# keep-starknet-strange/frieda

Measured on AMD Instinct MI355X. Metric: M31 field-elems/s committed (NTT+FRI+Merkle), higher is better.
Workload: dtype u32

## Files before the change

frieda_amd/csrc/clock_stamps.h:

```cpp
#pragma once

#ifdef FRIEDA_CLOCK_STAMPS
#define FR_CLOCK_SLOTS 16384
#define FR_CLOCK_DECL(name) __device__ unsigned long long name[4 * FR_CLOCK_SLOTS];
#define FR_CLOCK_BEGIN(tie)                                                                                                        \
    unsigned long long cs_c0_, cs_r0_;                                                                                             \
    asm volatile("s_memtime %0\n\ts_memrealtime %1\n\ts_waitcnt lgkmcnt(0)" : "=s"(cs_c0_), "=s"(cs_r0_)::"memory"); \
    asm volatile("" : "+v"(tie) : "s"(cs_c0_));
#define FR_CLOCK_END(buf, tie)                                                                                                     \
    {                                                                                                                              \
        asm volatile("" ::"v"(tie));                                                                                               \
        unsigned long long cs_c1_, cs_r1_;                                                                                         \
        asm volatile("s_memtime %0\n\ts_memrealtime %1\n\ts_waitcnt lgkmcnt(0)" : "=s"(cs_c1_), "=s"(cs_r1_)::"memory"); \
        if (threadIdx.x == 0 && blockIdx.y == 0 && blockIdx.z == 0 && blockIdx.x < FR_CLOCK_SLOTS) {                              \
            buf[4 * blockIdx.x + 0] = cs_c0_;                                                                                      \
            buf[4 * blockIdx.x + 1] = cs_r0_;                                                                                      \
            buf[4 * blockIdx.x + 2] = cs_c1_;                                                                                      \
            buf[4 * blockIdx.x + 3] = cs_r1_;                                                                                      \
        }                                                                                                                          \
    }
#define FR_CLOCK_READER(fn, buf)                                                                                                   \
    extern "C" int fn(unsigned long long* out, unsigned long n_words) {                                                            \
        const size_t bytes = sizeof(unsigned long long) * (n_words < 4 * FR_CLOCK_SLOTS ? n_words : 4 * FR_CLOCK_SLOTS);          \
        return hipMemcpyFromSymbol(out, HIP_SYMBOL(buf), bytes, 0, hipMemcpyDeviceToHost) == hipSuccess ? 0 : 1;                   \
    }
#else
#define FR_CLOCK_DECL(name)
#define FR_CLOCK_BEGIN(tie)
#define FR_CLOCK_END(buf, tie)
#define FR_CLOCK_READER(fn, buf)
#endif
```

frieda_amd/csrc/context.cpp:

```cpp
#include <cstring>
#include <cstdlib>
#include <string.h>

#include <cstdio>

#include <algorithm>
#include <mutex>

#include "host.h"

extern char** environ;

namespace frieda {

static constexpr uint32_t IDX_MASK = 0x7fffffffu;

CPoint point_from_index(uint32_t index) {
    static const std::array<CPoint, 31> pow2 = [] {
        std::array<CPoint, 31> t{};
        CPoint cur{CIRCLE_GEN_X, CIRCLE_GEN_Y};
        for (auto& e : t) {
            e = cur;
            cur = cp_double(cur);
        }
// ... 66 lines not shown
    auto* ti = reinterpret_cast<KernelTimerImpl*>(t);
    (void)hipEventRecord(ti->spans.back().stop, s);
}
}

k::Launch Ctx::launch() const {
    k::Launch l{stream, reinterpret_cast<k::KernelTimer*>(timer)};
    l.tune = &tuning;
    return l;
}

namespace k {
namespace {
struct KnobDesc {
    const char* name;
    long lo, hi;
    bool (*set)(Tuning&, long);
};
const KnobDesc KNOBS[] = {
    {"FRIEDA_T5_WIDE_LOG", 16, 24, [](Tuning& t, long v) { t.t5_wide_log = (uint32_t)v; return true; }},
    {"FRIEDA_T5_REG3_LOG", 0, 30, [](Tuning& t, long v) { t.t5_reg3_log = (uint32_t)v; return true; }},
    {"FRIEDA_T9_MAX_LOG", 8, 19, [](Tuning& t, long v) { t.t9_max_log = (uint32_t)v; return true; }},
    {"FRIEDA_TOP_MAX_LOG", 9, 11, [](Tuning& t, long v) { t.top_max_log = (uint32_t)v; return true; }},
    {"FRIEDA_NTT_CPW", 1, 4, [](Tuning& t, long v) {
         if (v == 4 && !t.lds_opt_in_ok) return false;
         t.ntt_cpw = (uint32_t)v;
         return true;
     }},
    {"FRIEDA_NTT_CPW_SMALL", 1, 4, [](Tuning& t, long v) { t.ntt_cpw_small = (uint32_t)v; return true; }},
    {"FRIEDA_NTT_REP", 0, 2, [](Tuning& t, long v) { t.ntt_rep = (uint32_t)v; return true; }},
    {"FRIEDA_NTT_NO_CP", 0, 1, [](Tuning& t, long v) { t.ntt_no_cp = v != 0; return true; }},
    {"FRIEDA_NTT_NO_PAD8", 0, 1, [](Tuning& t, long v) { t.ntt_no_pad8 = v != 0; return true; }},
    {"FRIEDA_NTT_PACKED_SRC", 0, 1, [](Tuning& t, long v) { t.ntt_packed_src = v != 0; return true; }},
    {"FRIEDA_NTT_TREE_REG_ONLY", 0, 1, [](Tuning& t, long v) { t.ntt_tree_reg_only = v != 0; return true; }},
    {"FRIEDA_NO_ENCODE_TREE_FUSION", 0, 1, [](Tuning& t, long v) { t.no_encode_tree_fusion = v != 0; return true; }},
    {"FRIEDA_ENCODE_TREE_FUSION_PROVE", 0, 1, [](Tuning& t, long v) { t.encode_tree_fusion_prove = v != 0; return true; }},
    {"FRIEDA_NO_SMALL_FUSED", 0, 1, [](Tuning& t, long v) { t.no_small_fused = v != 0; return true; }},
    {"FRIEDA_UNPACK_TILES", 1, 8, [](Tuning& t, long v) {
         if (v != 1 && v != 2 && v != 4 && v != 8) return false;
         t.unpack_tiles = (uint32_t)v;
         return true;
     }},
    {"FRIEDA_INTT_GENERIC", 0, 1, [](Tuning& t, long v) { t.intt_generic = v != 0; return true; }},
    {"FRIEDA_ERASURE_TREE_MIN_LOG", 6, 32, [](Tuning& t, long v) { t.erasure_tree_min_log = (uint32_t)v; return true; }},
    {"FRIEDA_TAIL_RUN_LOG", 4, 11, [](Tuning& t, long v) { t.tail_run_log = (uint32_t)v; return true; }},
    {"FRIEDA_HOST_DECOMMIT", 0, 1, [](Tuning& t, long v) { t.host_decommit = v != 0; return true; }},
    {"FRIEDA_GATHER_COPY", 0, 1, [](Tuning& t, long v) { t.gather_copy = v != 0; return true; }},
    {"FRIEDA_VERIFY_DEVICE_MIN", 0, 2147483648L, [](Tuning& t, long v) { t.verify_device_min = (uint32_t)v; return true; }},
    {"FRIEDA_OPEN_SMALL_MAX", 0, 512, [](Tuning& t, long v) { t.open_small_max = (uint32_t)v; return true; }},
    {"FRIEDA_TREE_SKIP_LOG", 10, 40, [](Tuning& t, long v) { t.tree_skip_log = (uint32_t)v; return true; }},
    {"FRIEDA_TREE_SKIP_LONE_LOG", 10, 40, [](Tuning& t, long v) { t.tree_skip_lone_log = (uint32_t)v; return true; }},
    {"FRIEDA_SEEDS_FOLD_GROUP", 0, 64, [](Tuning& t, long v) { t.seeds_fold_group = (uint32_t)v; return true; }},
    {"FRIEDA_TP_MIN_WGS", 0, 1 << 30, [](Tuning& t, long v) { t.tp_min_wgs = (uint32_t)v; return true; }},
    {"FRIEDA_GRIND_FRONT_WGS", 0, 2048, [](Tuning& t, long v) { t.grind_front_wgs = (uint32_t)v; return true; }},
    {"FRIEDA_GRIND_ITERS", 0, 64, [](Tuning& t, long v) { t.grind_iters = (uint32_t)v; return true; }},
    {"FRIEDA_BATCH_BUDGET_MB", 0, 262144, [](Tuning& t, long v) { t.batch_budget_mb = (uint32_t)v; return true; }},
    {"FRIEDA_BATCH_CALLS_PER_CTX", 1, 64, [](Tuning& t, long v) { t.batch_calls_per_ctx = (uint32_t)v; return true; }},
};
}

bool tuning_set(Tuning& t, const char* name, long value) {
    if (!name) return false;
    for (const KnobDesc& k : KNOBS) {
        if (strcmp(k.name, name) == 0) {
            if (value < k.lo || value > k.hi) return false;
            return k.set(t, value);
// ... 219 lines not shown
```

frieda_amd/csrc/kernels.h:

```cpp
#pragma once
#include <hip/hip_runtime.h>
#include <stddef.h>
#include <stdint.h>

#include "field.h"

namespace frieda {
namespace k {

inline size_t tw_level_offset(uint32_t n, uint32_t lv) { return ((size_t)1 << (n - 1)) - ((size_t)1 << (n - 1 - lv)); }
__device__ __forceinline__ size_t tw_level_offset_dev(uint32_t n, uint32_t lv) {
    return ((size_t)1 << (n - 1)) - ((size_t)1 << (n - 1 - lv));
}

struct KernelTimer;
struct Tuning {
    uint32_t t5_wide_log = 18;
    uint32_t t5_reg3_log = 0;
    uint32_t t9_max_log = 17;
    uint32_t top_max_log = 9;
    uint32_t ntt_cpw = 4;
    uint32_t ntt_cpw_small = 1;
    uint32_t ntt_rep = 2;
    bool ntt_no_pad8 = false;
    bool ntt_packed_src = true;
    bool ntt_no_cp = false;
    bool ntt_tree_reg_only = false;
    bool no_encode_tree_fusion = false;
    bool encode_tree_fusion_prove = false;
    bool no_small_fused = false;
    uint32_t unpack_tiles = 4;
    bool intt_generic = false;
    uint32_t erasure_tree_min_log = 15;
    uint32_t tail_run_log = 9;
    bool host_decommit = false;
    bool gather_copy = false;
    uint32_t verify_device_min = 1;
    uint32_t open_small_max = 512;
    uint32_t test_grind_first_log = 0;
    uint32_t batch_budget_mb = 0;
    uint32_t tree_skip_log = 18;
    uint32_t tree_skip_lone_log = 23;
    uint32_t tp_min_wgs = 768;
    uint32_t grind_iters = 0;
    uint32_t grind_front_wgs = 768;
    uint32_t seeds_fold_group = 0;
    uint32_t batch_calls_per_ctx = 1;
    uint64_t device_mem_bytes = 0;
    bool lds_opt_in_ok = true;
    uint64_t test_arena_limit = 0;
    uint64_t test_verify_pass_bytes = 0;
    bool test_poison = false;
    uint32_t test_poison_word = 0;
};
inline uint32_t tree_skip_threshold(const Tuning& t, uint32_t batch) {
    return batch >= 2 ? t.tree_skip_log : (t.tree_skip_lone_log > t.tree_skip_log ? t.tree_skip_lone_log : t.tree_skip_log);
}
Tuning tuning_from_env();
// ... 346 lines not shown
```

frieda_amd/csrc/ntt.hip:

```cpp
#include <hip/hip_runtime.h>

#include <type_traits>

#include <cstdlib>

#include "clock_stamps.h"
#include "kernels.h"
#include "tree_dev.h"

namespace frieda {
namespace k {

namespace {
using namespace treedev;

constexpr int NTT_THREADS = 256;
constexpr uint32_t TILE_LOG = 12;
#ifndef FRIEDA_NTT_PAD32
constexpr uint32_t TILE_WORDS = (1u << TILE_LOG) + (1u << (TILE_LOG - 4));
#else
constexpr uint32_t TILE_WORDS = (1u << TILE_LOG) + (1u << (TILE_LOG - 5));
#endif
constexpr uint32_t MAX_COLS_PER_WG = 4;
constexpr uint32_t MID_LOG_W = 4;

#ifndef FRIEDA_NTT_PAD32
__device__ __forceinline__ uint32_t pad(uint32_t e) { return e + (e >> 4); }
#else
__device__ __forceinline__ uint32_t pad(uint32_t e) { return e + (e >> 5); }
#endif
__device__ __forceinline__ uint32_t stage_group_base(uint32_t g, uint32_t lo) {
#ifdef FRIEDA_NTT_PAD32
    if (lo == 4) {
        const uint32_t t = g >> 4;
        const uint32_t h = (t & ~3u) | ((t & 1u) << 1) | ((t >> 1) & 1u);
        return (h << 8) | (g & 15u);
    }
#endif
    return ((g >> lo) << (lo + 4)) | (g & ((1u << lo) - 1));
}

#ifndef FRIEDA_NTT_IDLE
#define FRIEDA_NTT_IDLE 0x200
#endif
#ifndef FRIEDA_NTT_GROUP
#define FRIEDA_NTT_GROUP 8
#endif
#ifndef FRIEDA_NTT_GROUP_FUSED
#define FRIEDA_NTT_GROUP_FUSED 4
#endif
#ifndef FRIEDA_NTT_OUTER_PRIO
#define FRIEDA_NTT_OUTER_PRIO 3
#endif
__device__ __forceinline__ void ntt_enter() {
    if constexpr (FRIEDA_NTT_OUTER_PRIO != 0 && ((FRIEDA_NTT_IDLE >> 8) & 3) != 0) __builtin_amdgcn_s_setprio(FRIEDA_NTT_OUTER_PRIO);
}
template <int N, int G, int SET = -1>
// ... 97 lines not shown
                const uint32_t v = x[r];
                x[r] = m31_add(v, t);
                x[r | (1 << bit)] = m31_sub(v, t);
            }
        }
    }
}

__device__ __forceinline__ uint32_t circle_twiddle(const uint32_t* __restrict__ tw, uint32_t n, uint32_t h, uint32_t init_y) {
    if (n < 3) return (h & 1u) ? m31_neg(init_y) : init_y;
    uint32_t j = h >> 2, r = h & 3u;
    uint32_t v = tw[2 * j + (r < 2 ? 1 : 0)];
    return (r == 1 || r == 2) ? m31_neg(v) : v;
}

struct NttArgs {
    const uint32_t* in;
    size_t in_stride;
    uint32_t in_mask;
    uint32_t in_limit;
    uint32_t* out;
    size_t out_stride;
    const uint32_t* tw;
    uint32_t n, i_hi, i_lo, log_w, init_y;
    uint32_t ncols;
    uint32_t n_stages;
    uint32_t stage_r[3];
    size_t bstride_w;
    const uint8_t* pk;
    size_t pk_len;
    size_t pk_bstride;
    size_t pk_col_felts;
    uint32_t rep_log;
};

template <int R, int LO>
__device__ __forceinline__ void run_stage(uint32_t* lds, const NttArgs& a, uint32_t tb, uint32_t lo_rt, uint32_t hblk) {
    constexpr int E = 1 << R;
    const uint32_t lo = LO >= 0 ? (uint32_t)LO : lo_rt;
    const uint32_t n_groups = 1u << (tb - R);
    for (uint32_t g = threadIdx.x; g < n_groups; g += NTT_THREADS) {
        const uint32_t base = ((g >> lo) << (lo + R)) | (g & ((1u << lo) - 1));
        const uint32_t pbase = pad(base);
        uint32_t twd[E - 1];
#pragma unroll
        for (int q = 0; q < R; q++) {
            const uint32_t b = lo + R - 1 - q;
            const uint32_t i = a.i_lo + b - a.log_w;
            const uint32_t hbase = (hblk << (a.i_hi - i)) | (base >> (b + 1));
            if (i >= 1) {
                const uint32_t* lvl = a.tw + tw_level_offset_dev(a.n, i - 1) + hbase;
#pragma unroll
                for (int u = 0; u < (1 << q); u++) twd[(1 << q) - 1 + u] = lvl[u];
            } else {
#pragma unroll
                for (int u = 0; u < (1 << q); u++) twd[(1 << q) - 1 + u] = circle_twiddle(a.tw, a.n, hbase + (uint32_t)u, a.init_y);
            }
        }
        for (uint32_t c = 0; c < a.ncols; c++) {
            uint32_t* col = lds + c * TILE_WORDS + pbase;
            uint32_t x[E];
#pragma unroll
            for (int r = 0; r < E; r++) x[r] = col[pad((uint32_t)r << lo)];
#pragma unroll
            for (int q = 0; q < R; q++) {
                const int bit = R - 1 - q;
#pragma unroll
// ... 60 lines not shown
            run_stage<4, 4>(lds, a, tb, lo, hblk);
        else if (r == 4 && lo == 0)
            run_stage<4, 0>(lds, a, tb, lo, hblk);
        else if (r == 4)
            run_stage<4, -1>(lds, a, tb, lo, hblk);
        else if (r == 3)
            run_stage<3, -1>(lds, a, tb, lo, hblk);
        else if (r == 2)
            run_stage<2, -1>(lds, a, tb, lo, hblk);
        else
            run_stage<1, -1>(lds, a, tb, lo, hblk);
        top = lo;
        __syncthreads();
    }

    for (uint32_t c = 0; c < a.ncols; c++) {
        const uint32_t* col = lds + c * TILE_WORDS;
        uint32_t* dst = out + c * a.out_stride;
        if (vec) {
            for (uint32_t e = 4 * threadIdx.x; e < tile; e += 4 * NTT_THREADS) {
                uint32_t g = gbase | ((e >> a.log_w) << a.i_lo) | (e & wmask);
                uint32_t p = pad(e);
                *reinterpret_cast<uint4*>(dst + g) = make_uint4(col[p], col[p + 1], col[p + 2], col[p + 3]);
            }
        } else {
            for (uint32_t e = threadIdx.x; e < tile; e += NTT_THREADS) {
                uint32_t g = gbase | ((e >> a.log_w) << a.i_lo) | (e & wmask);
                dst[g] = col[pad(e)];
            }
        }
    }
}

template <int NS, int LOG_W>
__global__ __launch_bounds__(NTT_THREADS) void ntt_tile12_kernel(NttArgs a) {
    ntt_enter();
    __shared__ uint32_t lds[TILE_WORDS];
    const uint32_t g = threadIdx.x;
    const uint32_t nwb_log = a.i_lo - LOG_W;
    const uint32_t wblk = blockIdx.x & ((1u << nwb_log) - 1);
    const uint32_t hblk = blockIdx.x >> nwb_log;
    const uint32_t gbase = (hblk << (a.i_hi + 1)) | (wblk << LOG_W);
    constexpr uint32_t wmask = (1u << LOG_W) - 1;
    const size_t col0 = (size_t)blockIdx.y * a.ncols;
    const uint32_t* in = a.in + col0 * a.in_stride + blockIdx.z * a.bstride_w;
    uint32_t* out = a.out + col0 * a.out_stride + blockIdx.z * a.bstride_w;

    uint32_t pbase[NS];
    uint32_t twd[NS][15];
#pragma unroll
    for (int s = 0; s < NS; s++) {
        const uint32_t lo = 8 - 4 * s;
        const uint32_t base = stage_group_base(g, lo);
        pbase[s] = pad(base);
#pragma unroll
        for (int q = 0; q < 4; q++) {
            const uint32_t b = lo + 3 - q;
            const uint32_t i = a.i_lo + b - LOG_W;
            const uint32_t hbase = (hblk << (a.i_hi - i)) | (base >> (b + 1));
            if (LOG_W == 0 && s == NS - 1 && q == 3) {
#pragma unroll
                for (int u = 0; u < 8; u++) twd[s][7 + u] = 2u * circle_twiddle(a.tw, a.n, hbase + (uint32_t)u, a.init_y);
            } else {
                const uint32_t* lvl = a.tw + tw_level_offset_dev(a.n, i - 1) + hbase;
#pragma unroll
                for (int u = 0; u < (1 << q); u++) {
                    uint32_t v = lvl[u];
                    if (s == 0) v = (uint32_t)__builtin_amdgcn_readfirstlane((int)v);
                    twd[s][(1 << q) - 1 + u] = 2u * v;
                }
            }
        }
    }

    auto piece_e = [&](int kk) { return 4u * g + 1024u * (uint32_t)kk; };
    auto global_of = [&](uint32_t e) { return gbase | ((e >> LOG_W) << a.i_lo) | (e & wmask); };

    auto load4 = [&](const uint32_t* src, uint32_t gidx) {
        const uint32_t idx = gidx & a.in_mask;
        return idx < a.in_limit ? *reinterpret_cast<const uint4*>(src + idx) : make_uint4(0u, 0u, 0u, 0u);
    };
    uint4 pre[4];
#pragma unroll
    for (int kk = 0; kk < 4; kk++) pre[kk] = load4(in, global_of(piece_e(kk)));

    for (uint32_t c = 0; c < a.ncols; c++) {
#pragma unroll
        for (int kk = 0; kk < 4; kk++) {
            const uint32_t p = pad(piece_e(kk));
            lds[p] = pre[kk].x;
            lds[p + 1] = pre[kk].y;
            lds[p + 2] = pre[kk].z;
            lds[p + 3] = pre[kk].w;
        }
        __syncthreads();
        if (c + 1 < a.ncols) {
            const uint32_t* src = in + (size_t)(c + 1) * a.in_stride;
#pragma unroll
            for (int kk = 0; kk < 4; kk++) pre[kk] = load4(src, global_of(piece_e(kk)));
        }
        uint32_t x[16];
#pragma unroll
        for (int s = 0; s < NS; s++) {
            const uint32_t lo = 8 - 4 * s;
            uint32_t* col = lds + pbase[s];
#pragma unroll
            for (int r = 0; r < 16; r++) x[r] = col[pad((uint32_t)r << lo)];
            radix16_stage(x, twd[s]);
            if (s + 1 < NS || LOG_W != 0) {
#pragma unroll
                for (int r = 0; r < 16; r++) col[pad((uint32_t)r << lo)] = x[r];
            }
            if (LOG_W == 0 && NS == 3 && s == 1)
                __builtin_amdgcn_wave_barrier();
            else
                __syncthreads();
        }
        uint32_t* dst = out + (size_t)c * a.out_stride;
        if (LOG_W == 0) {
            uint4* o = reinterpret_cast<uint4*>(dst + gbase + 16u * g);
            o[0] = make_uint4(x[0], x[1], x[2], x[3]);
            o[1] = make_uint4(x[4], x[5], x[6], x[7]);
            o[2] = make_uint4(x[8], x[9], x[10], x[11]);
            o[3] = make_uint4(x[12], x[13], x[14], x[15]);
        } else {
#pragma unroll
            for (int kk = 0; kk < 4; kk++) {
                const uint32_t e = piece_e(kk), p = pad(e);
                *reinterpret_cast<uint4*>(dst + global_of(e)) = make_uint4(lds[p], lds[p + 1], lds[p + 2], lds[p + 3]);
            }
            __syncthreads();
        }
    }
}

struct PackedBlob {
    const uint8_t* p;
    uint32_t full;
    uint32_t tail;
};
__device__ __forceinline__ PackedBlob packed_blob(const uint8_t* __restrict__ p, size_t len) {
    PackedBlob b{p, (uint32_t)(len >> 2), 0u};
    for (size_t i = 4 * (size_t)b.full; i < len; i++) b.tail |= (uint32_t)p[i] << (8 * (i & 3));
    return b;
}
__device__ __forceinline__ uint32_t packed_dword(const PackedBlob& b, uint32_t d) {
    const bool in = d < b.full;
    const uint32_t v = *reinterpret_cast<const uint32_t*>(b.p + ((in ? d : 0u) << 2));
    return in ? v : (d == b.full ? b.tail : 0u);
}
__device__ __forceinline__ uint32_t packed_felt(const PackedBlob& b, uint32_t f) {
    const uint32_t d = (15u * f) >> 4, sh = (30u * f) & 31u;
    const uint64_t pair = ((uint64_t)packed_dword(b, d + 1) << 32) | packed_dword(b, d);
    return (uint32_t)(pair >> sh) & 0x3fffffffu;
}

template <int COLS, bool PACKED>
__global__ __launch_bounds__(NTT_THREADS) void ntt_tile12_rep_kernel(NttArgs a) {
    ntt_enter();
    constexpr int NS = 2;
    constexpr uint32_t LOG_W = MID_LOG_W;
    __shared__ uint32_t lds[TILE_WORDS];
    const uint32_t g = threadIdx.x;
    const uint32_t nwb_log = a.i_lo - LOG_W;
    const uint32_t wblk = blockIdx.x & ((1u << nwb_log) - 1);
    const uint32_t hblk0 = (blockIdx.x >> nwb_log) << a.rep_log;
    constexpr uint32_t wmask = (1u << LOG_W) - 1;
    const size_t col0 = (size_t)blockIdx.y * COLS;
    uint32_t* out = a.out + col0 * a.out_stride + blockIdx.z * a.bstride_w;

    auto piece_e = [&](int kk) { return 4u * g + 1024u * (uint32_t)kk; };
    auto low_of = [&](uint32_t e) { return (wblk << LOG_W) | ((e >> LOG_W) << a.i_lo) | (e & wmask); };

    const uint32_t e0 = stage_group_base(g, 8);
    uint32_t src[COLS][16];
    if constexpr (PACKED) {
        const PackedBlob blob = packed_blob(a.pk + blockIdx.z * a.pk_bstride, a.pk_len);
#pragma unroll
        for (int c = 0; c < COLS; c++) {
#pragma unroll
            for (int r = 0; r < 16; r++) {
                const uint32_t idx = low_of(e0 | ((uint32_t)r << 8)) & a.in_mask;
                const bool ok = idx < a.in_limit;
                const uint32_t v = packed_felt(blob, ok ? (uint32_t)((col0 + c) * a.pk_col_felts) + idx : 0u);
                src[c][r] = ok ? v : 0u;
            }
        }
    } else {
#pragma unroll
        for (int c = 0; c < COLS; c++) {
#pragma unroll
            for (int r = 0; r < 16; r++) {
                const uint32_t idx = low_of(e0 | ((uint32_t)r << 8)) & a.in_mask;
                src[c][r] = idx < a.in_limit ? (a.in + col0 * a.in_stride + blockIdx.z * a.bstride_w)[(size_t)c * a.in_stride + idx] : 0u;
            }
        }
    }
    uint32_t pbase[NS];
#pragma unroll
    for (int s = 0; s < NS; s++) {
        const uint32_t lo = 8 - 4 * s;
        pbase[s] = pad(stage_group_base(g, lo));
    }

#pragma unroll 1
    for (uint32_t h = 0; h < (1u << a.rep_log); h++) {
        const uint32_t hblk = hblk0 + h;
        const uint32_t gbase = hblk << (a.i_hi + 1);
        uint32_t twd[NS][15];
#pragma unroll
        for (int s = 0; s < NS; s++) {
            const uint32_t lo = 8 - 4 * s;
            const uint32_t base = stage_group_base(g, lo);
#pragma unroll
            for (int q = 0; q < 4; q++) {
                const uint32_t b = lo + 3 - q;
                const uint32_t i = a.i_lo + b - LOG_W;
                const uint32_t hbase = (hblk << (a.i_hi - i)) | (base >> (b + 1));
                const uint32_t* lvl = a.tw + tw_level_offset_dev(a.n, i - 1) + hbase;
#pragma unroll
                for (int u = 0; u < (1 << q); u++) {
                    uint32_t v = lvl[u];
                    if (s == 0) v = (uint32_t)__builtin_amdgcn_readfirstlane((int)v);
                    twd[s][(1 << q) - 1 + u] = 2u * v;
                }
            }
        }
#pragma unroll
        for (int c = 0; c < COLS; c++) {
            uint32_t x[16];
#pragma unroll
            for (int r = 0; r < 16; r++) x[r] = src[c][r];
#pragma unroll
            for (int s = 0; s < NS; s++) {
                const uint32_t lo = 8 - 4 * s;
                uint32_t* col = lds + pbase[s];
                if (s > 0) {
#pragma unroll
                    for (int r = 0; r < 16; r++) x[r] = col[pad((uint32_t)r << lo)];
                }
                radix16_stage(x, twd[s]);
#pragma unroll
                for (int r = 0; r < 16; r++) col[pad((uint32_t)r << lo)] = x[r];
                __syncthreads();
            }
            uint32_t* dst = out + (size_t)c * a.out_stride + gbase;
#pragma unroll
            for (int kk = 0; kk < 4; kk++) {
                const uint32_t e = piece_e(kk), p = pad(e);
                *reinterpret_cast<uint4*>(dst + low_of(e)) = make_uint4(lds[p], lds[p + 1], lds[p + 2], lds[p + 3]);
            }
            __syncthreads();
        }
    }
}

struct NttTreeArgs {
    NttArgs a;
    uint8_t* layers;
    uint8_t* last_out;
    size_t bstride;
};


template <bool STORE_ALL>
__device__ __forceinline__ void last_pass_four_columns(const NttArgs& a, uint32_t* lds, uint32_t g, uint32_t hblk, const uint32_t* in, uint32_t* out,
                                                       uint32_t (&v)[4][16]) {
    const uint32_t gbase = hblk << TILE_LOG;
    uint32_t pbase[3];
    uint32_t twd[3][15];
#pragma unroll
    for (int s = 0; s < 3; s++) {
        const uint32_t lo = 8 - 4 * s;
        const uint32_t base = stage_group_base(g, lo);
        pbase[s] = pad(base);
#pragma unroll
        for (int q = 0; q < 4; q++) {
            const uint32_t b = lo + 3 - q;
            const uint32_t hbase = (hblk << (11 - b)) | (base >> (b + 1));
            if (s == 2 && q == 3) {
#pragma unroll
                for (int u = 0; u < 8; u++) twd[s][7 + u] = 2u * circle_twiddle(a.tw, a.n, hbase + (uint32_t)u, a.init_y);
            } else {
                const uint32_t* lvl = a.tw + tw_level_offset_dev(a.n, b - 1) + hbase;
#pragma unroll
                for (int u = 0; u < (1 << q); u++) {
                    uint32_t v = lvl[u];
// ... 323 lines not shown
    const size_t i0 = e0 >> 1;
    const uint2 xy = *reinterpret_cast<const uint2*>(A.itw + 2 * (i0 >> 2));
    const uint32_t it0 = (i0 & 2) ? m31_neg(xy.x) : xy.y, it1 = (i0 & 2) ? xy.x : m31_neg(xy.y);
    const uint32_t il = A.itw[e0 >> 2];
    QM31 l1[2];
    l1[0] = qm_fold_pair(QM31{v[0][0], v[1][0], v[2][0], v[3][0]}, QM31{v[0][1], v[1][1], v[2][1], v[3][1]}, it0, am0);
    l1[1] = qm_fold_pair(QM31{v[0][2], v[1][2], v[2][2], v[3][2]}, QM31{v[0][3], v[1][3], v[2][3], v[3][3]}, it1, am0);
    const size_t s1 = (size_t)1 << (n - 1), s2 = (size_t)1 << (n - 2);
    uint32_t* d1 = A.line1 + i0;
    if (ACC) {
        const QM31 al = {A.alpha0[0], A.alpha0[1], A.alpha0[2], A.alpha0[3]};
        const QM31 asq = qm_mul(al, al);
        uint2 o[4];
#pragma unroll
        for (int cc = 0; cc < 4; cc++) o[cc] = *reinterpret_cast<const uint2*>(d1 + cc * s1);
        l1[0] = qm_add(qm_mul(QM31{o[0].x, o[1].x, o[2].x, o[3].x}, asq), l1[0]);
        l1[1] = qm_add(qm_mul(QM31{o[0].y, o[1].y, o[2].y, o[3].y}, asq), l1[1]);
    }
    *reinterpret_cast<uint2*>(d1) = make_uint2(l1[0].a, l1[1].a);
    *reinterpret_cast<uint2*>(d1 + s1) = make_uint2(l1[0].b, l1[1].b);
    *reinterpret_cast<uint2*>(d1 + 2 * s1) = make_uint2(l1[0].c, l1[1].c);
    *reinterpret_cast<uint2*>(d1 + 3 * s1) = make_uint2(l1[0].d, l1[1].d);
    const QM31 l2 = qm_fold_pair(l1[0], l1[1], il, am1);
    uint32_t* d2 = A.line2 + (e0 >> 2);
    d2[0] = l2.a;
    d2[s2] = l2.b;
    d2[2 * s2] = l2.c;
    d2[3 * s2] = l2.d;
}

}

FR_CLOCK_READER(frieda_debug_clock_ntt_last_tree, g_clock_ntt_last_tree)

namespace {
uint32_t evaluate_plan(const Launch& L_, const uint32_t* d_coef, size_t coef_stride, uint32_t ncols, uint32_t L, uint32_t n, uint32_t out_log,
                       const uint32_t* d_tw, DomainScalars ds, uint32_t* d_out, size_t out_stride, const EncodeTreeSink* sink,
                       const EncodeFoldSink* fsink = nullptr, const BlobSource* blob = nullptr);
}

void circle_evaluate(const Launch& L_, const uint32_t* d_coef, size_t coef_stride, uint32_t ncols, uint32_t L, uint32_t n,
                     const uint32_t* d_tw, DomainScalars ds, uint32_t* d_out, size_t out_stride) {
    (void)evaluate_plan(L_, d_coef, coef_stride, ncols, L, n, n, d_tw, ds, d_out, out_stride, nullptr);
}

void circle_evaluate_prefix(const Launch& L_, const uint32_t* d_coef, size_t coef_stride, uint32_t ncols, uint32_t L, uint32_t n, uint32_t out_log,
                            const uint32_t* d_tw, DomainScalars ds, uint32_t* d_out, size_t out_stride) {
    (void)evaluate_plan(L_, d_coef, coef_stride, ncols, L, n, out_log < L ? L : (out_log > n ? n : out_log), d_tw, ds, d_out, out_stride, nullptr);
}

uint32_t circle_evaluate_into_tree(const Launch& L_, const uint32_t* d_coef, size_t coef_stride, uint32_t ncols, uint32_t L, uint32_t n,
                               const uint32_t* d_tw, DomainScalars ds, uint32_t* d_out, size_t out_stride, const EncodeTreeSink* sink,
                               const BlobSource* blob) {
    return evaluate_plan(L_, d_coef, coef_stride, ncols, L, n, n, d_tw, ds, d_out, out_stride, sink, nullptr, blob);
}

hipError_t ntt_opt_in_dynamic_lds() {
    const int bytes = (int)(MAX_COLS_PER_WG * TILE_WORDS * sizeof(uint32_t));
    hipError_t e = hipFuncSetAttribute(reinterpret_cast<const void*>(ntt_tile_kernel), hipFuncAttributeMaxDynamicSharedMemorySize, bytes);
    if (e != hipSuccess) return e;
    e = hipFuncSetAttribute(reinterpret_cast<const void*>(ntt_last_fold_cp_kernel<false>), hipFuncAttributeMaxDynamicSharedMemorySize, bytes);
    if (e != hipSuccess) return e;
    return hipFuncSetAttribute(reinterpret_cast<const void*>(ntt_last_fold_cp_kernel<true>), hipFuncAttributeMaxDynamicSharedMemorySize, bytes);
}

bool circle_evaluate_fold2(const Launch& L_, const uint32_t* d_coef, size_t coef_stride, uint32_t L, uint32_t n, const uint32_t* d_tw,
// ... 19 lines not shown
    bool blob_pending = blob != nullptr;
    auto unpack_now = [&]() {
        unpack30(L_, blob->bytes, blob->len, const_cast<uint32_t*>(d_coef), blob->n_padded, blob->bstride);
        blob_pending = false;
    };
    const double enc_bytes = 4.0 * ncols * ((double)N + (double)((size_t)1 << L));
    if (L == 0) {
        if (blob_pending) unpack_now();
        Scope scope(L_, "ntt_broadcast", enc_bytes);
        dim3 grid((unsigned)((N + 255) / 256), ncols, L_.batch);
        ntt_broadcast_kernel<<<grid, 256, 0, s>>>(d_coef, coef_stride, d_out, out_stride, N, L_.bstride / 4);
        return 0;
    }
    const uint32_t cpw_max = L_.tune->ntt_cpw <= MAX_COLS_PER_WG ? L_.tune->ntt_cpw : MAX_COLS_PER_WG;
    uint32_t cpw = cpw_max;
    while (ncols % cpw) cpw--;
    const size_t lds_bytes = (size_t)cpw * TILE_WORDS * sizeof(uint32_t);

    const uint32_t last_t = L < TILE_LOG ? L : TILE_LOG;
    uint32_t rest = L - last_t;
    const uint32_t mid_max = TILE_LOG - MID_LOG_W;
    const uint32_t n_mid_generic = (rest + mid_max - 1) / mid_max;
    uint32_t n_mid_fast = 0;
    NttArgs a{};
    a.in = d_coef;
    a.in_stride = coef_stride;
    a.in_mask = (uint32_t)(((size_t)1 << L) - 1);
    a.out = d_out;
    a.out_stride = out_stride;
    a.tw = d_tw;
    a.n = n;
    a.init_y = ds.init_y;
    a.bstride_w = L_.bstride / 4;
    uint32_t cpw4 = MAX_COLS_PER_WG;
    const uint32_t cpw_small = L_.tune->ntt_cpw_small;
    if ((N >> TILE_LOG) * (size_t)L_.batch < 512) cpw4 = cpw_small;
    while (ncols % cpw4) cpw4--;
    uint32_t fused_levels = 0;
    auto launch_pass = [&](uint32_t t, const char* name) {
        const bool aligned = ((a.in_stride | a.out_stride) & 3) == 0 && (a.in_mask & 3u) == 3u &&
                             ((reinterpret_cast<uintptr_t>(a.in) | reinterpret_cast<uintptr_t>(a.out) | L_.bstride) & 15) == 0;
        const uint32_t hb_log = n - 1 - a.i_hi;
        const uint64_t rep_wgs = (uint64_t)((N >> TILE_LOG) >> (hb_log < 3 ? hb_log : 3)) * (ncols / 2) * L_.batch;
        const bool use_rep = L_.tune->ntt_rep == 1 || (L_.tune->ntt_rep == 2 && rep_wgs >= 1024);
        const bool rep = use_rep && out_log == n && aligned && t == 8 && a.log_w == MID_LOG_W && hb_log >= 1 && ((uint64_t)a.in_mask >> (a.i_hi + 1)) == 0 && ncols % 2 == 0;
        bool packed = false;
        if (blob_pending) {
            packed = rep && L_.tune->ntt_packed_src && blob->len >= 4 && blob->len <= ((size_t)1 << 30) &&
                     (uint64_t)ncols * coef_stride <= ((uint64_t)1 << 28) && (reinterpret_cast<uintptr_t>(blob->bytes) & 3) == 0 &&
                     (L_.batch == 1 || (blob->bstride & 3) == 0);
            if (packed)
                blob_pending = false;
            else
                unpack_now();
        }
        if (sink && aligned && a.log_w == 0 && t == 12 && ncols == 4 && n >= TILE_LOG && out_log == n) {
            NttTreeArgs ta{};
            ta.a = a;
            ta.a.ncols = 4;
            ta.layers = sink->layers;
            ta.last_out = sink->last_out;
            ta.bstride = L_.bstride;
            const bool reg_only = L_.tune->ntt_tree_reg_only;
            const uint32_t levels = reg_only ? 5u : ENCODE_TREE_LEVELS;
            double bytes = enc_bytes / ((n_mid_fast ? n_mid_fast : n_mid_generic) + 1) + 48.0 * (double)N;
            for (uint32_t l = 1; l < levels; l++) bytes += 96.0 * (double)(N >> l);
// ... 18 lines not shown
#undef FR_LAUNCH_LAST_TREE
            fused_levels = levels;
            return;
        }
        if (fsink && aligned && a.log_w == 0 && t == 12 && ncols == 4 && n >= TILE_LOG + 2 && out_log == n && L_.batch == 1 &&
            ((reinterpret_cast<uintptr_t>(fsink->line1) | reinterpret_cast<uintptr_t>(fsink->line2) | reinterpret_cast<uintptr_t>(fsink->itw)) & 15) == 0) {
            NttFoldArgs fa{};
            fa.a = a;
            fa.a.ncols = 4;
            fa.itw = fsink->itw;
            fa.inv_init_y = ds.inv_init_y;
            for (int i = 0; i < 4; i++) fa.alpha0[i] = fsink->alpha0[i], fa.alpha1[i] = fsink->alpha1[i];
            fa.line1 = fsink->line1;
            fa.line2 = fsink->line2;
            Scope scope(L_, "ntt_last_fold2", enc_bytes / ((n_mid_fast ? n_mid_fast : n_mid_generic) + 1) + 36.0 * (double)N);
            const dim3 grid((unsigned)(N >> TILE_LOG), 1, 1);
            const bool side_by_side = (N >> TILE_LOG) < 512 && L_.tune->lds_opt_in_ok && L_.tune->ntt_cpw == 4 && !L_.tune->ntt_no_cp;
            const size_t cp_lds = (size_t)4 * TILE_WORDS * sizeof(uint32_t);
            if (side_by_side && fsink->accumulate)
                ntt_last_fold_cp_kernel<true><<<grid, NTT_CP_THREADS, cp_lds, s>>>(fa);
            else if (side_by_side)
                ntt_last_fold_cp_kernel<false><<<grid, NTT_CP_THREADS, cp_lds, s>>>(fa);
            else if (fsink->accumulate)
                ntt_last_fold_kernel<true><<<grid, NTT_THREADS, 0, s>>>(fa);
            else
                ntt_last_fold_kernel<false><<<grid, NTT_THREADS, 0, s>>>(fa);
            fused_levels = 1;
            return;
        }
        Scope scope(L_, name, enc_bytes / ((n_mid_fast ? n_mid_fast : n_mid_generic) + 1));
        if (rep) {
            a.rep_log = hb_log < 3 ? hb_log : 3;
            a.ncols = 2;
            dim3 grid((unsigned)((N >> TILE_LOG) >> a.rep_log), ncols / 2, L_.batch);
            if (packed) {
                a.pk = blob->bytes;
                a.pk_len = blob->len;
                a.pk_bstride = L_.batch > 1 ? blob->bstride : 0;
                a.pk_col_felts = coef_stride;
                ntt_tile12_rep_kernel<2, true><<<grid, NTT_THREADS, 0, s>>>(a);
            } else {
                ntt_tile12_rep_kernel<2, false><<<grid, NTT_THREADS, 0, s>>>(a);
            }
            a.rep_log = 0;
        } else if (aligned && t + a.log_w == TILE_LOG && (t == 12 || t == 8 || t == 4)) {
            a.ncols = cpw4;
            dim3 grid((unsigned)(N >> TILE_LOG), ncols / cpw4, L_.batch);
            if (t == 12)
                ntt_tile12_kernel<3, 0><<<grid, NTT_THREADS, 0, s>>>(a);
            else if (t == 8)
                ntt_tile12_kernel<2, MID_LOG_W><<<grid, NTT_THREADS, 0, s>>>(a);
            else
                ntt_tile12_kernel<1, 8><<<grid, NTT_THREADS, 0, s>>>(a);
        } else {
            a.ncols = cpw;
            set_stages(a, t);
            dim3 grid((unsigned)(N >> (t + a.log_w)), ncols / cpw, L_.batch);
            ntt_tile_kernel<<<grid, NTT_THREADS, lds_bytes, s>>>(a);
        }
    };
    a.in_limit = a.in_mask + 1;
    uint32_t i_hi = L - 1;
    const bool no_pad8 = L_.tune->ntt_no_pad8;
    const uint32_t units = (rest + 3) / 4, padz = 4 * units - rest;
    const bool base_aligned = ((a.in_stride | a.out_stride) & 3) == 0 &&
                              ((reinterpret_cast<uintptr_t>(a.in) | reinterpret_cast<uintptr_t>(a.out) | L_.bstride) & 15) == 0;
    if (rest > 0 && base_aligned && padz <= out_log - L && L >= 4 && (!no_pad8 || (padz == 0 && (units & 1) == 0))) {
        n_mid_fast = (units + 1) / 2;
        uint32_t top = L - 1 + padz, left = units;
        bool first = true;
        while (left) {
            const uint32_t t = (left & 1) ? 4u : 8u;
            a.i_hi = top;
            a.i_lo = top + 1 - t;
            a.log_w = TILE_LOG - t;
            if (first) {
                a.in_mask = (uint32_t)(((size_t)1 << (L + padz)) - 1);
                a.in_limit = (uint32_t)1 << L;
            }
            launch_pass(t, "ntt_pass_mid");
            a.in = d_out;
            a.in_stride = out_stride;
            a.in_mask = (uint32_t)(N - 1);
// ... 33 lines not shown
```

Baseline: 49.07 billion.

## Batch multiple blobs per workgroup in last NTT tile and prefetch rep twiddles

The last radix-16x3 tile kernel can now process several batch blobs per workgroup. It reuses the per-thread twiddles loaded once and prefetches the next blob's input while computing the current one, with the blob count chosen automatically to keep enough workgroups. The rep kernel stages the next high-block's twiddles into shared memory during the current block's work instead of reloading them from global memory at each iteration. This cuts repeated twiddle loads and launch-level parallelism in exchange for longer-running workgroups and extra LDS traffic. Clock-stamp instrumentation macros are also added, but they are compiled out by default.

```diff
diff --git a/frieda_amd/csrc/clock_stamps.h b/frieda_amd/csrc/clock_stamps.h
--- a/frieda_amd/csrc/clock_stamps.h
+++ b/frieda_amd/csrc/clock_stamps.h
@@ -19,6 +19,25 @@
             buf[4 * blockIdx.x + 3] = cs_r1_;                                                                                      \
         }                                                                                                                          \
     }
+#define FR_CLOCK_VAR(var) unsigned long long var = 0;
+#define FR_CLOCK_NOW(var, after, before)                                                                          \
+    {                                                                                                             \
+        asm volatile("s_memtime %0\n\ts_waitcnt lgkmcnt(0)" : "=s"(var) : "v"(after) : "memory");                 \
+        asm volatile("" : "+v"(before) : "s"(var));                                                               \
+    }
+#define FR_CLOCK_ADD(acc, t1, t0) acc += t1 - t0;
+#define FR_CLOCK_END4(buf, tie, w1, w2)                                                                           \
+    {                                                                                                             \
+        asm volatile("" ::"v"(tie));                                                                              \
+        unsigned long long cs_c1_;                                                                                \
+        asm volatile("s_memtime %0\n\ts_waitcnt lgkmcnt(0)" : "=s"(cs_c1_)::"memory");                            \
+        if (threadIdx.x == 0 && blockIdx.y == 0 && blockIdx.z == 0 && blockIdx.x < FR_CLOCK_SLOTS) {             \
+            buf[4 * blockIdx.x + 0] = cs_c0_;                                                                     \
+            buf[4 * blockIdx.x + 1] = w1;                                                                         \
+            buf[4 * blockIdx.x + 2] = w2;                                                                         \
+            buf[4 * blockIdx.x + 3] = cs_c1_;                                                                     \
+        }                                                                                                         \
+    }
 #define FR_CLOCK_READER(fn, buf)                                                                                                   \
     extern "C" int fn(unsigned long long* out, unsigned long n_words) {                                                            \
         const size_t bytes = sizeof(unsigned long long) * (n_words < 4 * FR_CLOCK_SLOTS ? n_words : 4 * FR_CLOCK_SLOTS);          \
@@ -28,5 +47,9 @@
 #define FR_CLOCK_DECL(name)
 #define FR_CLOCK_BEGIN(tie)
 #define FR_CLOCK_END(buf, tie)
+#define FR_CLOCK_VAR(var)
+#define FR_CLOCK_NOW(var, after, before)
+#define FR_CLOCK_ADD(acc, t1, t0)
+#define FR_CLOCK_END4(buf, tie, w1, w2)
 #define FR_CLOCK_READER(fn, buf)
 #endif
diff --git a/frieda_amd/csrc/context.cpp b/frieda_amd/csrc/context.cpp
--- a/frieda_amd/csrc/context.cpp
+++ b/frieda_amd/csrc/context.cpp
@@ -122,6 +122,8 @@
     {"FRIEDA_NTT_NO_CP", 0, 1, [](Tuning& t, long v) { t.ntt_no_cp = v != 0; return true; }},
     {"FRIEDA_NTT_NO_PAD8", 0, 1, [](Tuning& t, long v) { t.ntt_no_pad8 = v != 0; return true; }},
     {"FRIEDA_NTT_PACKED_SRC", 0, 1, [](Tuning& t, long v) { t.ntt_packed_src = v != 0; return true; }},
+    {"FRIEDA_NTT_LAST_BLOBS", 0, 1024, [](Tuning& t, long v) { t.ntt_last_blobs = (uint32_t)v; return true; }},
+    {"FRIEDA_NTT_REP_TW_AHEAD", 0, 1, [](Tuning& t, long v) { t.ntt_rep_tw_ahead = v != 0; return true; }},
     {"FRIEDA_NTT_TREE_REG_ONLY", 0, 1, [](Tuning& t, long v) { t.ntt_tree_reg_only = v != 0; return true; }},
     {"FRIEDA_NO_ENCODE_TREE_FUSION", 0, 1, [](Tuning& t, long v) { t.no_encode_tree_fusion = v != 0; return true; }},
     {"FRIEDA_ENCODE_TREE_FUSION_PROVE", 0, 1, [](Tuning& t, long v) { t.encode_tree_fusion_prove = v != 0; return true; }},
diff --git a/frieda_amd/csrc/kernels.h b/frieda_amd/csrc/kernels.h
--- a/frieda_amd/csrc/kernels.h
+++ b/frieda_amd/csrc/kernels.h
@@ -24,6 +24,8 @@
     uint32_t ntt_rep = 2;
     bool ntt_no_pad8 = false;
     bool ntt_packed_src = true;
+    uint32_t ntt_last_blobs = 0;
+    bool ntt_rep_tw_ahead = true;
     bool ntt_no_cp = false;
     bool ntt_tree_reg_only = false;
     bool no_encode_tree_fusion = false;
diff --git a/frieda_amd/csrc/ntt.hip b/frieda_amd/csrc/ntt.hip
--- a/frieda_amd/csrc/ntt.hip
+++ b/frieda_amd/csrc/ntt.hip
@@ -23,6 +23,7 @@
 #endif
 constexpr uint32_t MAX_COLS_PER_WG = 4;
 constexpr uint32_t MID_LOG_W = 4;
+constexpr uint32_t LAST_BLOBS_AUTO = 5;
 
 #ifndef FRIEDA_NTT_PAD32
 __device__ __forceinline__ uint32_t pad(uint32_t e) { return e + (e >> 4); }
@@ -186,7 +187,29 @@
     size_t pk_bstride;
     size_t pk_col_felts;
     uint32_t rep_log;
+    uint32_t batch;
+    uint32_t blobs_per_wg;
+    uint32_t tw_ahead;
 };
+
+constexpr uint32_t SHARED_TW_WORDS = 255;
+__device__ __forceinline__ uint32_t shared_twiddle_word(const NttArgs& a, uint32_t hblk, uint32_t w) {
+    const uint32_t s = w >= 15u ? 1u : 0u;
+    const uint32_t h = s ? (w - 15u) / 15u : 0u;
+    const uint32_t j = s ? w - 15u - 15u * h : w;
+    const uint32_t q = 31u - (uint32_t)__clz((int)(j + 1u)), u = j + 1u - (1u << q);
+    const uint32_t i = a.i_hi - 4u * s - q;
+    const uint32_t hbase = ((s ? (hblk << 4) | h : hblk) << q) + u;
+    return 2u * a.tw[tw_level_offset_dev(a.n, i - 1) + hbase];
+}
+__device__ __forceinline__ void shared_twiddles_read(const uint32_t* tws, uint32_t g, uint32_t (&tw0)[15], uint32_t (&tw1)[15]) {
+    const uint32_t* mine = tws + 15u + 15u * (stage_group_base(g, 4) >> 8);
+#pragma unroll
+    for (int j = 0; j < 15; j++) {
+        tw0[j] = (uint32_t)__builtin_amdgcn_readfirstlane((int)tws[j]);
+        tw1[j] = mine[j];
+    }
+}
 
 template <int R, int LO>
 __device__ __forceinline__ void run_stage(uint32_t* lds, const NttArgs& a, uint32_t tb, uint32_t lo_rt, uint32_t hblk) {
@@ -313,19 +336,40 @@
     }
 }
 
-template <int NS, int LOG_W>
-__global__ __launch_bounds__(NTT_THREADS) void ntt_tile12_kernel(NttArgs a) {
-    ntt_enter();
-    __shared__ uint32_t lds[TILE_WORDS];
-    const uint32_t g = threadIdx.x;
+FR_CLOCK_DECL(g_clock_ntt_last)
+FR_CLOCK_DECL(g_clock_ntt_rep)
+template <int NS, int LOG_W, bool MANY>
+__device__ __forceinline__ void tile12_columns(const NttArgs& a, uint32_t* lds) {
+    uint32_t g_tie = threadIdx.x;
+    FR_CLOCK_BEGIN(g_tie)
+    FR_CLOCK_VAR(cs_first)
+    const uint32_t g = g_tie;
     const uint32_t nwb_log = a.i_lo - LOG_W;
     const uint32_t wblk = blockIdx.x & ((1u << nwb_log) - 1);
     const uint32_t hblk = blockIdx.x >> nwb_log;
     const uint32_t gbase = (hblk << (a.i_hi + 1)) | (wblk << LOG_W);
     constexpr uint32_t wmask = (1u << LOG_W) - 1;
     const size_t col0 = (size_t)blockIdx.y * a.ncols;
-    const uint32_t* in = a.in + col0 * a.in_stride + blockIdx.z * a.bstride_w;
-    uint32_t* out = a.out + col0 * a.out_stride + blockIdx.z * a.bstride_w;
+    uint32_t z0 = blockIdx.z, nb = 1;
+    if constexpr (MANY) {
+        z0 = blockIdx.z * a.blobs_per_wg;
+        nb = a.batch - z0 < a.blobs_per_wg ? a.batch - z0 : a.blobs_per_wg;
+    }
+    const uint32_t* in = a.in + col0 * a.in_stride + z0 * a.bstride_w;
+    uint32_t* out = a.out + col0 * a.out_stride + z0 * a.bstride_w;
+
+    auto piece_e = [&](int kk) { return 4u * g + 1024u * (uint32_t)kk; };
+    auto global_of = [&](uint32_t e) { return gbase | ((e >> LOG_W) << a.i_lo) | (e & wmask); };
+
+    auto load4 = [&](const uint32_t* src, uint32_t gidx) {
+        const uint32_t idx = gidx & a.in_mask;
+        return idx < a.in_limit ? *reinterpret_cast<const uint4*>(src + idx) : make_uint4(0u, 0u, 0u, 0u);
+    };
+    uint4 pre[4];
+    if constexpr (MANY) {
+#pragma unroll
+        for (int kk = 0; kk < 4; kk++) pre[kk] = load4(in, global_of(piece_e(kk)));
+    }
 
     uint32_t pbase[NS];
     uint32_t twd[NS][15];
@@ -353,66 +397,85 @@
             }
         }
     }
-
-    auto piece_e = [&](int kk) { return 4u * g + 1024u * (uint32_t)kk; };
-    auto global_of = [&](uint32_t e) { return gbase | ((e >> LOG_W) << a.i_lo) | (e & wmask); };
-
-    auto load4 = [&](const uint32_t* src, uint32_t gidx) {
-        const uint32_t idx = gidx & a.in_mask;
-        return idx < a.in_limit ? *reinterpret_cast<const uint4*>(src + idx) : make_uint4(0u, 0u, 0u, 0u);
-    };
-    uint4 pre[4];
-#pragma unroll
-    for (int kk = 0; kk < 4; kk++) pre[kk] = load4(in, global_of(piece_e(kk)));
-
-    for (uint32_t c = 0; c < a.ncols; c++) {
-#pragma unroll
-        for (int kk = 0; kk < 4; kk++) {
-            const uint32_t p = pad(piece_e(kk));
-            lds[p] = pre[kk].x;
-            lds[p + 1] = pre[kk].y;
-            lds[p + 2] = pre[kk].z;
-            lds[p + 3] = pre[kk].w;
-        }
-        __syncthreads();
-        if (c + 1 < a.ncols) {
-            const uint32_t* src = in + (size_t)(c + 1) * a.in_stride;
-#pragma unroll
-            for (int kk = 0; kk < 4; kk++) pre[kk] = load4(src, global_of(piece_e(kk)));
-        }
-        uint32_t x[16];
-#pragma unroll
-        for (int s = 0; s < NS; s++) {
-            const uint32_t lo = 8 - 4 * s;
-            uint32_t* col = lds + pbase[s];
-#pragma unroll
-            for (int r = 0; r < 16; r++) x[r] = col[pad((uint32_t)r << lo)];
-            radix16_stage(x, twd[s]);
-            if (s + 1 < NS || LOG_W != 0) {
-#pragma unroll
-                for (int r = 0; r < 16; r++) col[pad((uint32_t)r << lo)] = x[r];
-            }
-            if (LOG_W == 0 && NS == 3 && s == 1)
-                __builtin_amdgcn_wave_barrier();
-            else
+    if constexpr (!MANY) {
+#pragma unroll
+        for (int kk = 0; kk < 4; kk++) pre[kk] = load4(in, global_of(piece_e(kk)));
+    }
+
+    for (uint32_t bi = 0; bi < nb; bi++) {
+        for (uint32_t c = 0; c < a.ncols; c++) {
+#pragma unroll
+            for (int kk = 0; kk < 4; kk++) {
+                const uint32_t p = pad(piece_e(kk));
+                lds[p] = pre[kk].x;
+                lds[p + 1] = pre[kk].y;
+                lds[p + 2] = pre[kk].z;
+                lds[p + 3] = pre[kk].w;
+            }
+            __syncthreads();
+            const bool more_cols = c + 1 < a.ncols;
+            if (more_cols || (MANY && bi + 1 < nb)) {
+                const uint32_t* src = more_cols ? in + (size_t)(c + 1) * a.in_stride : in + a.bstride_w;
+#pragma unroll
+                for (int kk = 0; kk < 4; kk++) pre[kk] = load4(src, global_of(piece_e(kk)));
+            }
+            uint32_t x[16];
+#pragma unroll
+            for (int s = 0; s < NS; s++) {
+                const uint32_t lo = 8 - 4 * s;
+                uint32_t* col = lds + pbase[s];
+#pragma unroll
+                for (int r = 0; r < 16; r++) x[r] = col[pad((uint32_t)r << lo)];
+#ifdef FRIEDA_CLOCK_STAMPS
+                if (NS == 3 && LOG_W == 0 && s == 0 && bi == 0 && c == 0) FR_CLOCK_NOW(cs_first, x[15], x[0])
+#endif
+                radix16_stage(x, twd[s]);
+                if (s + 1 < NS || LOG_W != 0) {
+#pragma unroll
+                    for (int r = 0; r < 16; r++) col[pad((uint32_t)r << lo)] = x[r];
+                }
+                if (LOG_W == 0 && NS == 3 && s == 1)
+                    __builtin_amdgcn_wave_barrier();
+                else
+                    __syncthreads();
+            }
+            uint32_t* dst = out + (size_t)c * a.out_stride;
+            if (LOG_W == 0) {
+                uint4* o = reinterpret_cast<uint4*>(dst + gbase + 16u * g);
+                o[0] = make_uint4(x[0], x[1], x[2], x[3]);
+                o[1] = make_uint4(x[4], x[5], x[6], x[7]);
+                o[2] = make_uint4(x[8], x[9], x[10], x[11]);
+                o[3] = make_uint4(x[12], x[13], x[14], x[15]);
+#ifdef FRIEDA_CLOCK_STAMPS
+                if (NS == 3 && bi + 1 == nb && c + 1 == a.ncols) FR_CLOCK_END4(g_clock_ntt_last, x[15], cs_first, 0ull)
+#endif
+            } else {
+#pragma unroll
+                for (int kk = 0; kk < 4; kk++) {
+                    const uint32_t e = piece_e(kk), p = pad(e);
+                    *reinterpret_cast<uint4*>(dst + global_of(e)) = make_uint4(lds[p], lds[p + 1], lds[p + 2], lds[p + 3]);
+                }
                 __syncthreads();
-        }
-        uint32_t* dst = out + (size_t)c * a.out_stride;
-        if (LOG_W == 0) {
-            uint4* o = reinterpret_cast<uint4*>(dst + gbase + 16u * g);
-            o[0] = make_uint4(x[0], x[1], x[2], x[3]);
-            o[1] = make_uint4(x[4], x[5], x[6], x[7]);
-            o[2] = make_uint4(x[8], x[9], x[10], x[11]);
-            o[3] = make_uint4(x[12], x[13], x[14], x[15]);
-        } else {
-#pragma unroll
-            for (int kk = 0; kk < 4; kk++) {
-                const uint32_t e = piece_e(kk), p = pad(e);
-                *reinterpret_cast<uint4*>(dst + global_of(e)) = make_uint4(lds[p], lds[p + 1], lds[p + 2], lds[p + 3]);
-            }
-            __syncthreads();
-        }
-    }
+            }
+        }
+        if constexpr (MANY) {
+            in += a.bstride_w;
+            out += a.bstride_w;
+        }
+    }
+}
+
+template <int NS, int LOG_W>
+__global__ __launch_bounds__(NTT_THREADS) void ntt_tile12_kernel(NttArgs a) {
+    ntt_enter();
+    __shared__ uint32_t lds[TILE_WORDS];
+    if constexpr (NS == 3 && LOG_W == 0) {
+        if (a.blobs_per_wg > 1) {
+            tile12_columns<NS, LOG_W, true>(a, lds);
+            return;
+        }
+    }
+    tile12_columns<NS, LOG_W, false>(a, lds);
 }
 
 struct PackedBlob {
@@ -442,7 +505,13 @@
     constexpr int NS = 2;
     constexpr uint32_t LOG_W = MID_LOG_W;
     __shared__ uint32_t lds[TILE_WORDS];
-    const uint32_t g = threadIdx.x;
+    uint32_t g_tie = threadIdx.x;
+    FR_CLOCK_BEGIN(g_tie)
+    FR_CLOCK_VAR(cs_first)
+    FR_CLOCK_VAR(cs_top)
+    FR_CLOCK_VAR(cs_go)
+    FR_CLOCK_VAR(cs_wait)
+    const uint32_t g = g_tie;
     const uint32_t nwb_log = a.i_lo - LOG_W;
     const uint32_t wblk = blockIdx.x & ((1u << nwb_log) - 1);
     const uint32_t hblk0 = (blockIdx.x >> nwb_log) << a.rep_log;
@@ -483,57 +552,87 @@
         const uint32_t lo = 8 - 4 * s;
         pbase[s] = pad(stage_group_base(g, lo));
     }
+    __shared__ uint32_t tws[NTT_THREADS];
+    auto high_blocks = [&](auto ahead_c) {
+        constexpr bool ahead = decltype(ahead_c)::value;
+        const uint32_t tw_w = g < SHARED_TW_WORDS ? g : SHARED_TW_WORDS - 1;
+        if constexpr (ahead) {
+            tws[g] = shared_twiddle_word(a, hblk0, tw_w);
+            __syncthreads();
+        }
 
 #pragma unroll 1
-    for (uint32_t h = 0; h < (1u << a.rep_log); h++) {
-        const uint32_t hblk = hblk0 + h;
-        const uint32_t gbase = hblk << (a.i_hi + 1);
-        uint32_t twd[NS][15];
-#pragma unroll
-        for (int s = 0; s < NS; s++) {
-            const uint32_t lo = 8 - 4 * s;
-            const uint32_t base = stage_group_base(g, lo);
-#pragma unroll
-            for (int q = 0; q < 4; q++) {
-                const uint32_t b = lo + 3 - q;
-                const uint32_t i = a.i_lo + b - LOG_W;
-                const uint32_t hbase = (hblk << (a.i_hi - i)) | (base >> (b + 1));
-                const uint32_t* lvl = a.tw + tw_level_offset_dev(a.n, i - 1) + hbase;
-#pragma unroll
-                for (int u = 0; u < (1 << q); u++) {
-                    uint32_t v = lvl[u];
-                    if (s == 0) v = (uint32_t)__builtin_amdgcn_readfirstlane((int)v);
-                    twd[s][(1 << q) - 1 + u] = 2u * v;
+        for (uint32_t h = 0; h < (1u << a.rep_log); h++) {
+            const uint32_t hblk = hblk0 + h;
+            const uint32_t gbase = hblk << (a.i_hi + 1);
+            FR_CLOCK_NOW(cs_top, src[0][0], src[0][0])
+            uint32_t twd[NS][15];
+            uint32_t tw_next = 0;
+            if constexpr (ahead) {
+                shared_twiddles_read(tws, g, twd[0], twd[1]);
+                if (h + 1 < (1u << a.rep_log)) tw_next = shared_twiddle_word(a, hblk + 1, tw_w);
+            }
+            if constexpr (!ahead) {
+#pragma unroll
+                for (int s = 0; s < NS; s++) {
+                    const uint32_t lo = 8 - 4 * s;
+                    const uint32_t base = stage_group_base(g, lo);
+#pragma unroll
+                    for (int q = 0; q < 4; q++) {
+                        const uint32_t b = lo + 3 - q;
+                        const uint32_t i = a.i_lo + b - LOG_W;
+                        const uint32_t hbase = (hblk << (a.i_hi - i)) | (base >> (b + 1));
+                        const uint32_t* lvl = a.tw + tw_level_offset_dev(a.n, i - 1) + hbase;
+#pragma unroll
+                        for (int u = 0; u < (1 << q); u++) {
+                            uint32_t v = lvl[u];
+                            if (s == 0) v = (uint32_t)__builtin_amdgcn_readfirstlane((int)v);
+                            twd[s][(1 << q) - 1 + u] = 2u * v;
+                        }
+                    }
                 }
             }
-        }
-#pragma unroll
-        for (int c = 0; c < COLS; c++) {
-            uint32_t x[16];
-#pragma unroll
-            for (int r = 0; r < 16; r++) x[r] = src[c][r];
-#pragma unroll
-            for (int s = 0; s < NS; s++) {
-                const uint32_t lo = 8 - 4 * s;
-                uint32_t* col = lds + pbase[s];
-                if (s > 0) {
-#pragma unroll
-                    for (int r = 0; r < 16; r++) x[r] = col[pad((uint32_t)r << lo)];
+#pragma unroll
+            for (int c = 0; c < COLS; c++) {
+                uint32_t x[16];
+#pragma unroll
+                for (int r = 0; r < 16; r++) x[r] = src[c][r];
+#ifdef FRIEDA_CLOCK_STAMPS
+                if (c == 0) {
+                    FR_CLOCK_NOW(cs_go, twd[1][14], x[0])
+                    FR_CLOCK_ADD(cs_wait, cs_go, cs_top)
+                    if (h == 0) cs_first = cs_go;
                 }
-                radix16_stage(x, twd[s]);
-#pragma unroll
-                for (int r = 0; r < 16; r++) col[pad((uint32_t)r << lo)] = x[r];
+#endif
+#pragma unroll
+                for (int s = 0; s < NS; s++) {
+                    const uint32_t lo = 8 - 4 * s;
+                    uint32_t* col = lds + pbase[s];
+                    if (s > 0) {
+#pragma unroll
+                        for (int r = 0; r < 16; r++) x[r] = col[pad((uint32_t)r << lo)];
+                    }
+                    radix16_stage(x, twd[s]);
+#pragma unroll
+                    for (int r = 0; r < 16; r++) col[pad((uint32_t)r << lo)] = x[r];
+                    __syncthreads();
+                }
+                uint32_t* dst = out + (size_t)c * a.out_stride + gbase;
+#pragma unroll
+                for (int kk = 0; kk < 4; kk++) {
+                    const uint32_t e = piece_e(kk), p = pad(e);
+                    *reinterpret_cast<uint4*>(dst + low_of(e)) = make_uint4(lds[p], lds[p + 1], lds[p + 2], lds[p + 3]);
+                }
+                if (c == COLS - 1 && ahead) tws[g] = tw_next;
                 __syncthreads();
             }
-            uint32_t* dst = out + (size_t)c * a.out_stride + gbase;
-#pragma unroll
-            for (int kk = 0; kk < 4; kk++) {
-                const uint32_t e = piece_e(kk), p = pad(e);
-                *reinterpret_cast<uint4*>(dst + low_of(e)) = make_uint4(lds[p], lds[p + 1], lds[p + 2], lds[p + 3]);
-            }
-            __syncthreads();
-        }
-    }
+        }
+        FR_CLOCK_END4(g_clock_ntt_rep, g_tie, cs_first, cs_wait)
+    };
+    if (a.tw_ahead)
+        high_blocks(std::true_type{});
+    else
+        high_blocks(std::false_type{});
 }
 
 struct NttTreeArgs {
@@ -923,6 +1022,8 @@
 }
 
 FR_CLOCK_READER(frieda_debug_clock_ntt_last_tree, g_clock_ntt_last_tree)
+FR_CLOCK_READER(frieda_debug_clock_ntt_last, g_clock_ntt_last)
+FR_CLOCK_READER(frieda_debug_clock_ntt_rep, g_clock_ntt_rep)
 
 namespace {
 uint32_t evaluate_plan(const Launch& L_, const uint32_t* d_coef, size_t coef_stride, uint32_t ncols, uint32_t L, uint32_t n, uint32_t out_log,
@@ -1008,6 +1109,8 @@
     a.n = n;
     a.init_y = ds.init_y;
     a.bstride_w = L_.bstride / 4;
+    a.batch = L_.batch;
+    a.blobs_per_wg = 1;
     uint32_t cpw4 = MAX_COLS_PER_WG;
     const uint32_t cpw_small = L_.tune->ntt_cpw_small;
     if ((N >> TILE_LOG) * (size_t)L_.batch < 512) cpw4 = cpw_small;
@@ -1092,6 +1195,7 @@
         if (rep) {
             a.rep_log = hb_log < 3 ? hb_log : 3;
             a.ncols = 2;
+            a.tw_ahead = L_.tune->ntt_rep_tw_ahead ? 1u : 0u;
             dim3 grid((unsigned)((N >> TILE_LOG) >> a.rep_log), ncols / 2, L_.batch);
             if (packed) {
                 a.pk = blob->bytes;
@@ -1103,12 +1207,24 @@
                 ntt_tile12_rep_kernel<2, false><<<grid, NTT_THREADS, 0, s>>>(a);
             }
             a.rep_log = 0;
+            a.tw_ahead = 0;
         } else if (aligned && t + a.log_w == TILE_LOG && (t == 12 || t == 8 || t == 4)) {
             a.ncols = cpw4;
             dim3 grid((unsigned)(N >> TILE_LOG), ncols / cpw4, L_.batch);
-            if (t == 12)
+            if (t == 12) {
+                const uint64_t tiles = N >> TILE_LOG;
+                if (L_.batch > 1 && tiles * L_.batch >= 512) {
+                    uint32_t bpw = L_.tune->ntt_last_blobs;
+                    if (bpw == 0) {
+                        bpw = LAST_BLOBS_AUTO;
+                        while (bpw > 1 && tiles * (ncols / cpw4) * ((L_.batch + bpw - 1) / bpw) < 8192) bpw--;
+                    }
+                    a.blobs_per_wg = bpw < L_.batch ? bpw : L_.batch;
+                    grid.z = (L_.batch + a.blobs_per_wg - 1) / a.blobs_per_wg;
+                }
                 ntt_tile12_kernel<3, 0><<<grid, NTT_THREADS, 0, s>>>(a);
-            else if (t == 8)
+                a.blobs_per_wg = 1;
+            } else if (t == 8)
                 ntt_tile12_kernel<2, MID_LOG_W><<<grid, NTT_THREADS, 0, s>>>(a);
             else
                 ntt_tile12_kernel<1, 8><<<grid, NTT_THREADS, 0, s>>>(a);
```

Result: no change. 49.39 billion, median of 6 (+0.6%).
